# ChunLI-666/PointCloudProcessor

Measured on AMD Instinct MI355X. Metric: Mpoints×frames/sec colorized, higher is better.
Workload: dtype f32/f64

## Files before the change

### include/pcp_hip.h

```cpp
#ifndef PCP_HIP_H
#define PCP_HIP_H

#include <stdint.h>

#ifdef __cplusplus
extern "C" {
#endif

#define PCP_ABI_VERSION 6

#define PCP_OK 0
#define PCP_ERR_INVALID (-1)
#define PCP_ERR_STATE (-2)
#define PCP_ERR_DEVICE (-3)
#define PCP_ERR_NOMEM (-4)
#define PCP_ERR_RANGE (-5)

typedef struct pcp_context pcp_context;

typedef struct pcp_pose {
  double x, y, z, qw, qx, qy, qz;
} pcp_pose;

typedef struct pcp_camera {
// ... 107 lines not shown
int pcp_colour_smooth_local_packed(pcp_context *ctx, float radius, const uint32_t *in_rgba, uint32_t *out_rgba,
                                   int64_t *out_has_count);

int pcp_mls_process(pcp_context *ctx, const pcp_mls_params *p, int64_t *out_count);
int pcp_mls_process_shard(pcp_context *ctx, const pcp_mls_params *p, int64_t index_begin, int64_t index_end,
                          int64_t *out_count);
int pcp_mls_process_slab(pcp_context *ctx, const pcp_mls_params *p, int32_t slab, int32_t n_slabs, int64_t *out_count);
int pcp_mls_stream_begin(pcp_context *ctx, const pcp_mls_params *p, int64_t chunk_capacity, int64_t *out_total,
                         int32_t *out_chunks);
int pcp_mls_stream_next(pcp_context *ctx, int64_t *out_count);
int pcp_mls_stream_seek(pcp_context *ctx, int32_t chunk);
int pcp_mls_fetch(pcp_context *ctx, int64_t capacity, float *out_xyz, float *out_normal, float *out_curvature,
                  int32_t *out_index);
int pcp_cloud_smooth(pcp_context *ctx, const pcp_mls_params *p, int64_t *out_count);

int pcp_cloud_smooth_stream_begin(pcp_context *ctx, const pcp_mls_params *p, int64_t chunk_capacity, int64_t *out_total_rows,
                                  int64_t *out_kept_rows, int32_t *out_chunks);
int pcp_cloud_smooth_stream_next(pcp_context *ctx, int64_t *out_count);
int pcp_cloud_smooth_stream_end(pcp_context *ctx);
int pcp_cloud_smooth_stream_stats(pcp_context *ctx, double out[13]);
int pcp_sor(pcp_context *ctx, int32_t mean_k, double std_mul, uint8_t *out_keep, int64_t *out_kept);
int64_t pcp_sor_chunk_points(void);
int pcp_sor_partial(pcp_context *ctx, int32_t mean_k, int32_t slab, int32_t n_slabs, int64_t capacity, double *out_chunk_sums,
                    int64_t *out_first_chunk, int64_t *out_chunks);
int pcp_sor_finish(pcp_context *ctx, double std_mul, const double *all_chunk_sums, int64_t n_chunks, int32_t slab, int32_t n_slabs,
                   uint8_t *out_keep, int64_t *out_kept);

int pcp_upload_intensity(pcp_context *ctx, const float *intensity, int64_t n);
int pcp_nid_prepare(pcp_context *ctx, int64_t *out_points);
int pcp_nid_evaluate(pcp_context *ctx, const double T[16], const double *T_init, int32_t bins, double *cost,
                     double grad6[6], int32_t *valid);
int pcp_nid_optimize(pcp_context *ctx, const double T_init[16], int32_t bins, int32_t max_outer_iterations,
                     double T_out[16], double *final_cost, int32_t *evaluations);

int pcp_nid_accumulate(pcp_context *ctx, const double T[16], int32_t bins);
int pcp_nid_histograms_device(pcp_context *ctx, void **device_ptr, int64_t *count);
int pcp_nid_finish(pcp_context *ctx, int32_t bins, double *cost, double grad6[6], int32_t *valid);
typedef int (*pcp_nid_eval_fn)(void *user, const double T[16], int32_t bins, double *cost, double grad6[6], int32_t *valid);
int pcp_nid_optimize_with(pcp_context *ctx, pcp_nid_eval_fn eval, void *user, const double T_init[16], int32_t bins,
                          int32_t max_outer_iterations, double T_out[16], double *final_cost, int32_t *evaluations);

int pcp_close_pairs(pcp_context *ctx, double radius, int64_t *points_with_close_neighbour);

int pcp_timing_enable(pcp_context *ctx, int32_t on);
int pcp_timing_reset(pcp_context *ctx);
int pcp_timing_get(pcp_context *ctx, int32_t kernel_id, double *total_ms, int64_t *launches);
const char *pcp_kernel_name(int32_t kernel_id);
int pcp_tile_mask_density(pcp_context *ctx, double *kept_fraction);
int pcp_tile_masks(pcp_context *ctx, int64_t *tiles, int32_t *mask_words, uint32_t *out_words);
int pcp_sor_redo_fraction(pcp_context *ctx, double *fraction);
int pcp_sor_distances(pcp_context *ctx, int64_t capacity, float *out_distance);
int pcp_selftest_arithmetic(pcp_context *ctx, int64_t samples, uint64_t seed, int64_t *mismatches_fp64,
                            int64_t *mismatches_fp32);

#ifdef __cplusplus
}
#endif
#endif
```

### pointcloudprocessor_amd/capi.py

```python
from __future__ import annotations

import ctypes as C
import os
import re

import numpy as np

from . import _build

PCP_OK = 0
PCP_ERR_INVALID = -1
PCP_ERR_STATE = -2
PCP_ERR_DEVICE = -3
PCP_ERR_NOMEM = -4
PCP_ERR_RANGE = -5

NID_EVAL_FN = C.CFUNCTYPE(C.c_int, C.c_void_p, C.POINTER(C.c_double), C.c_int32, C.POINTER(C.c_double), C.POINTER(C.c_double),
                          C.POINTER(C.c_int32))
K_PROJECT, K_DEPTH, K_COLOUR, K_VISIBILITY, K_MLS_GRID, K_MLS_FIT, K_MISC, K_SOR, K_MLS_VOXEL, K_TILE_MASK, K_NID, K_HPR = range(12)
K_COLOUR_SMOOTH = 12
K_COUNT = 13


class PcpError(RuntimeError):
# ... 536 lines not shown
        valid = C.c_int32()
        self._check(self.lib.pcp_nid_finish(self.h, C.c_int32(bins), C.byref(cost), _ptr(grad), C.byref(valid)))
        return cost.value, grad, bool(valid.value)

    def nid_optimize_with(self, evaluate, T_init, bins: int = 16, max_outer_iterations: int = 10):
        errors = []

        @NID_EVAL_FN
        def trampoline(_user, T, b, cost, grad, valid):
            try:
                c, g, ok = evaluate(np.ctypeslib.as_array(T, (16,)).copy().reshape(4, 4), int(b))
                cost[0] = float(c)
                for k in range(6):
                    grad[k] = float(g[k])
                valid[0] = 1 if ok else 0
                return 0
            except Exception as e:
                errors.append(e)
                return -3

        Ti = np.ascontiguousarray(T_init, np.float64).reshape(16)
        out = np.zeros(16, np.float64)
        cost = C.c_double()
        evals = C.c_int32()
        rc = self.lib.pcp_nid_optimize_with(self.h, trampoline, None, _ptr(Ti), C.c_int32(bins), C.c_int32(max_outer_iterations),
                                            _ptr(out), C.byref(cost), C.byref(evals))
        if errors:
            raise errors[0]
        self._check(rc)
        return out.reshape(4, 4), cost.value, evals.value

    def timing_enable(self, on: bool = True):
        self._check(self.lib.pcp_timing_enable(self.h, C.c_int32(1 if on else 0)))

    def timing_reset(self):
        self._check(self.lib.pcp_timing_reset(self.h))

    def timing_get(self, kernel_id: int):
        ms = C.c_double()
        cnt = C.c_int64()
        self._check(self.lib.pcp_timing_get(self.h, C.c_int32(kernel_id), C.byref(ms), C.byref(cnt)))
        return ms.value, cnt.value

    def tile_mask_density(self) -> float:
        v = C.c_double()
        self._check(self.lib.pcp_tile_mask_density(self.h, C.byref(v)))
        return v.value

    def selftest_arithmetic(self, samples: int = 1 << 26, seed: int = 1):
        a, b = C.c_int64(), C.c_int64()
        self._check(self.lib.pcp_selftest_arithmetic(self.h, C.c_int64(samples), C.c_uint64(seed), C.byref(a), C.byref(b)))
        return a.value, b.value

    def tile_masks(self) -> np.ndarray:
        t, w = C.c_int64(), C.c_int32()
        self._check(self.lib.pcp_tile_masks(self.h, C.byref(t), C.byref(w), None))
        out = np.empty((t.value, w.value), np.uint32)
        self._check(self.lib.pcp_tile_masks(self.h, None, None, _ptr(out)))
        return out

    def kernel_name(self, kernel_id: int) -> str:
        return self.lib.pcp_kernel_name(C.c_int32(kernel_id)).decode()
```

### pointcloudprocessor_amd/csrc/pcp_colour.hip

```cpp
#include <algorithm>
#include <cfloat>
#include <cstdlib>

#include "pcp_device.hpp"
#include "pcp_hsv.hpp"
#include "pcp_scan.hpp"

namespace pcp {

constexpr int kBlock = 256;
constexpr uint32_t kFltMaxBits = 0x7f7fffffu;

template <bool kCommon>
__device__ __forceinline__ DevCamera common_camera(const DevCamera &in) {
  DevCamera c = in;
  if constexpr (kCommon) {
    c.cull_mode = PCP_CULL_ZBUFFER;
    c.enable_zbuf = 1;
    c.pretest = 1;
    c.ds_fast = 1;
  }
  return c;
}
inline bool is_common_camera(const DevCamera &c) {
// ... 290 lines not shown
  constexpr uint32_t kXcd = 8, kSuper = kXcd * kXcdChunk;
  const uint32_t b = blockIdx.x;
  if (b >= (gridDim.x / kSuper) * kSuper) return b;
  const uint32_t x = b % kXcd, slot = b / kXcd;
  return ((slot / kXcdChunk) * kXcd + x) * kXcdChunk + slot % kXcdChunk;
}

constexpr unsigned long long kDepthEmpty = 0x7f7f7f7f7f7f7f7full;
__device__ __forceinline__ void depth_min(unsigned long long *__restrict__ map, int32_t cell, unsigned long long bits) {
  if (bits < map[cell]) atomicMin(map + cell, bits);
}
__device__ __forceinline__ double sumsq64(float xc, float yc, float zc) {
  const double X = xc, Y = yc, Z = zc;
  return (X * X + Y * Y) + Z * Z;
}
__global__ __launch_bounds__(kBlock) void k_depth_finish(const unsigned long long *__restrict__ sq, int64_t count,
                                                         uint32_t *__restrict__ range) {
  int64_t i = static_cast<int64_t>(blockIdx.x) * kBlock + threadIdx.x;
  const int64_t stride = static_cast<int64_t>(gridDim.x) * kBlock;
  for (; i < count; i += stride) {
    const unsigned long long b = sq[i];
    float r = FLT_MAX;
    if (b != kDepthEmpty) r = fminf(static_cast<float>(sqrt(__longlong_as_double(static_cast<long long>(b)))), FLT_MAX);
    range[i] = __float_as_uint(r);
  }
}

__device__ __forceinline__ uint32_t range_bits(int32_t w, int32_t f0, int32_t f1) {
  const int32_t fb = max(f0, w << 5), fe = min(f1, (w << 5) + 32);
  const int32_t nb = fe - fb;
  return nb <= 0 ? 0u : (((nb >= 32) ? 0xffffffffu : ((1u << nb) - 1u)) << (fb & 31));
}

template <bool kCommon>
__global__ __launch_bounds__(kBlock) void k_depth_pass(const float *__restrict__ x, const float *__restrict__ y,
                                                       const float *__restrict__ z, int64_t n, DevCamera cam_in,
                                                       const DevFrame *__restrict__ frames, int32_t f0, int32_t f1,
                                                       unsigned long long *__restrict__ depth, int64_t cells,
                                                       int32_t depth_first_frame, uint32_t *__restrict__ tile_mask,
                                                       const uint32_t *__restrict__ tile_inside, int32_t words,
                                                       const int32_t *__restrict__ tile_order) {
  DevCamera cam = common_camera<kCommon>(cam_in);
  if constexpr (kCommon) cam.pretest = 0;
  __shared__ unsigned long long combine[kBlock];
  const int lane = threadIdx.x & 63;
  unsigned long long *tbl = combine + (threadIdx.x & ~63);
  const int64_t j = tile_order ? static_cast<int64_t>(tile_order[blockIdx.x]) * 64 + threadIdx.x
                               : static_cast<int64_t>(xcd_chunked_block()) * kBlock + threadIdx.x;
  const bool live = j < n;
  if (!__ballot(live)) return;
  const float px = live ? x[j] : 0.0f, py = live ? y[j] : 0.0f, pz = live ? z[j] : 0.0f;
  const int64_t tile = __builtin_amdgcn_readfirstlane(static_cast<int32_t>(j >> 6));
  const bool finite_sure = cam.frames_bounded != 0 && __all(fabsf(px) <= 0x1p40f && fabsf(py) <= 0x1p40f && fabsf(pz) <= 0x1p40f);
  unsigned long long *held_at = nullptr;
  unsigned long long held_bits = 0ull, held_seen = 0ull;
  auto settle_held = [&]() {
    if (held_at && held_bits < held_seen) atomicMin(held_at, held_bits);
    held_at = nullptr;
  };
  for (int32_t w = f0 >> 5; w <= (f1 - 1) >> 5; ++w) {
    const uint32_t in_range = range_bits(w, f0, f1);
    uint32_t todo = in_range;
    if (tile_mask) todo &= tile_mask[tile * words + w];
    todo = __builtin_amdgcn_readfirstlane(todo);
    const uint32_t inside = tile_inside ? __builtin_amdgcn_readfirstlane(tile_inside[tile * words + w]) : 0u;
    uint32_t seen = 0u;
    while (todo) {
      const int32_t b = __builtin_ctz(todo);
      const int32_t f = (w << 5) + b;
      todo &= todo - 1u;
      const DevFrame &fr = frames[f];
      const Projected p = project_point(cam, fr.w2c, px, py, pz, ((inside >> b) & 1u) == 0u, finite_sure);
      const bool in_map = live && p.cell >= 0;
      const bool cand = live && p.pixel >= 0 && (cam.enable_zbuf ? p.cell >= 0 : p.cell != -1);
      if (__ballot(cand)) seen |= 1u << b;
      settle_held();
      if (cam.enable_zbuf && __ballot(in_map)) {
        unsigned long long *map = depth + static_cast<uint64_t>(static_cast<uint32_t>(f - depth_first_frame)) * static_cast<uint32_t>(cells);
        unsigned long long key = ~0ull, sbits = 0ull;
        if (in_map) {
          sbits = static_cast<unsigned long long>(__double_as_longlong(sumsq64(p.xc, p.yc, p.zc)));
          key = (static_cast<unsigned long long>(static_cast<uint32_t>(p.cell)) << 32) | (sbits >> 32);
        }
        tbl[lane] = ~0ull;
        __builtin_amdgcn_wave_barrier();
        if (in_map) atomicMin(&tbl[p.cell & 63], key);
        __builtin_amdgcn_wave_barrier();
        if (in_map) {
          const unsigned long long got = tbl[p.cell & 63];
          if (got == key || static_cast<uint32_t>(got >> 32) != static_cast<uint32_t>(p.cell)) {
            held_at = map + p.cell;
            held_bits = sbits;
            held_seen = *held_at;
          }
        }
        __builtin_amdgcn_wave_barrier();
      }
    }
    if (tile_mask && lane == 0 && live) {
      uint32_t *dst = tile_mask + tile * words + w;
      *dst = (*dst & ~in_range) | seen;
    }
  }
  settle_held();
}

__global__ __launch_bounds__(kBlock) void k_visibility(const float *__restrict__ x, const float *__restrict__ y,
                                                       const float *__restrict__ z, int64_t n, DevCamera cam,
                                                       DevFrame fr, const uint32_t *__restrict__ depth,
                                                       const int32_t *__restrict__ perm,
                                                       uint8_t *__restrict__ keep, int32_t require_pixel) {
  const int64_t i = static_cast<int64_t>(blockIdx.x) * kBlock + threadIdx.x;
  if (i >= n) return;
  const Projected p = project_point(cam, fr.w2c, x[i], y[i], z[i]);
  bool k = keep_rule(cam, p, depth);
  if (require_pixel) k = k && p.pixel >= 0;
  if (k) keep[perm ? perm[i] : i] = 1;
}

__device__ __forceinline__ bool keep_by_depth(float xc, float yc, float zc, double lim) {
  const double s = sumsq64(xc, yc, zc);
  const double L = lim * lim;
  bool keep = s < L * (1.0 - 0x1p-40);
  const bool sure = lim > 0.0 && (keep || s > L * (1.0 + 0x1p-40));
  if (!sure) keep = !(sqrt(s) > lim);
  return keep;
}

struct TopState {
  float *score;
  uint32_t *rgb;
  int32_t *frame;
  int32_t *count;
};

struct MatchArgs {
  const uint8_t *in_a;
  unsigned long long *moved;
  float e2;
};

template <bool kCommon, int kMatch, bool kOneShot>
__global__ __launch_bounds__(kBlock) void k_colour_pass(const float *__restrict__ x, const float *__restrict__ y,
                                                        const float *__restrict__ z, int64_t n, DevCamera cam_in,
                                                        const DevFrame *__restrict__ frames, int32_t f0, int32_t f1,
                                                        const uint32_t *__restrict__ depth, int64_t cells,
                                                        const uint32_t *__restrict__ tile_mask, int32_t words,
                                                        const uint32_t *__restrict__ images, int64_t image_px,
                                                        TopState st, const int32_t *__restrict__ perm,
                                                        uint32_t *__restrict__ rgba, int32_t flags_in,
                                                        const uint32_t *__restrict__ hull_bits_in, MatchArgs mb) {
  DevCamera cam = common_camera<kCommon>(cam_in);
  if constexpr (kMatch == 1) cam.match_mode = PCP_MATCH_IDENTITY;
  if constexpr (kMatch == 2 || kMatch == 3) cam.match_mode = PCP_MATCH_ROUNDTRIP;
  const uint32_t *__restrict__ hull_bits = kCommon ? nullptr : hull_bits_in;
  const int32_t flags = kOneShot ? 4 : flags_in;
  const int64_t j = static_cast<int64_t>(xcd_chunked_block()) * kBlock + threadIdx.x;
  const bool live = j < n;
  if (!__ballot(live)) return;
  const float px = live ? x[j] : 0.0f, py = live ? y[j] : 0.0f, pz = live ? z[j] : 0.0f;
  const int64_t tile = __builtin_amdgcn_readfirstlane(static_cast<int32_t>(j >> 6));
  const bool finite_sure = cam.frames_bounded != 0 && __all(fabsf(px) <= 0x1p40f && fabsf(py) <= 0x1p40f && fabsf(pz) <= 0x1p40f);
  Top5 t;
  t.init();
  if ((flags & 1) && live) {
    t.s0 = st.score[0 * n + j]; t.s1 = st.score[1 * n + j]; t.s2 = st.score[2 * n + j];
    t.s3 = st.score[3 * n + j]; t.s4 = st.score[4 * n + j];
    t.c0 = st.rgb[0 * n + j]; t.c1 = st.rgb[1 * n + j]; t.c2 = st.rgb[2 * n + j];
    t.c3 = st.rgb[3 * n + j]; t.c4 = st.rgb[4 * n + j];
    t.f0 = st.frame[0 * n + j]; t.f1 = st.frame[1 * n + j]; t.f2 = st.frame[2 * n + j];
    t.f3 = st.frame[3 * n + j]; t.f4 = st.frame[4 * n + j];
    t.count = st.count[j];
  }
  [[maybe_unused]] bool in_a = false;
  [[maybe_unused]] uint32_t moved = 0u;
  if constexpr (kMatch == 3) in_a = live && mb.in_a[j] != 0;
  for (int32_t w = f0 >> 5; w <= (f1 - 1) >> 5; ++w) {
    uint32_t todo = range_bits(w, f0, f1);
    if (tile_mask) todo &= tile_mask[tile * words + w];
    todo = __builtin_amdgcn_readfirstlane(todo);
    const uint32_t hull_word = (hull_bits && live) ? hull_bits[static_cast<int64_t>(w) * n + j] : 0xffffffffu;
    while (todo) {
      const int32_t f = (w << 5) + __builtin_ctz(todo);
      todo &= todo - 1u;
      const DevFrame &fr = frames[f];
      const Projected p = project_point<false>(cam, fr.w2c, px, py, pz, true, finite_sure);
      const bool cand = live && p.pixel >= 0 && (cam.enable_zbuf ? p.cell >= 0 : p.cell != -1) &&
                        ((hull_word >> (f & 31)) & 1u);
      if (cand) {
        const uint32_t dbits = cam.enable_zbuf ? depth[static_cast<uint64_t>(static_cast<uint32_t>(f)) * static_cast<uint32_t>(cells) + static_cast<uint32_t>(p.cell)] : 0u;
        bool keep = true;
        if (cam.enable_zbuf) keep = keep_by_depth(p.xc, p.yc, p.zc, static_cast<double>(__uint_as_float(dbits)) + cam.slack);
        float sx = p.xc, sy = p.yc, sz = p.zc;
        if constexpr (kMatch == 3) {
          if (keep) keep = roundtrip_sample_moved(cam, fr, px, py, pz, sx, sy, sz, mb.e2, moved) && !in_a;
        } else {
          if (cam.match_mode == PCP_MATCH_ROUNDTRIP && keep) keep = roundtrip_sample(cam, fr, px, py, pz, sx, sy, sz);
        }
        if (keep) {
          const uint32_t texel = images[static_cast<uint64_t>(static_cast<uint32_t>(f)) * static_cast<uint32_t>(image_px) + static_cast<uint32_t>(p.pixel)];
          t.insert(final_score(sx, sy, sz, fr.px, fr.py, fr.pz), texel & 0xffffffu, f);
        }
      }
    }
  }
  if constexpr (kMatch == 3) {
    if (moved) atomicAdd(mb.moved, static_cast<unsigned long long>(moved));
  }
  if (!live) return;
  if (flags & 2) {
    st.score[0 * n + j] = t.s0; st.score[1 * n + j] = t.s1; st.score[2 * n + j] = t.s2;
    st.score[3 * n + j] = t.s3; st.score[4 * n + j] = t.s4;
    st.rgb[0 * n + j] = t.c0; st.rgb[1 * n + j] = t.c1; st.rgb[2 * n + j] = t.c2;
    st.rgb[3 * n + j] = t.c3; st.rgb[4 * n + j] = t.c4;
    st.frame[0 * n + j] = t.f0; st.frame[1 * n + j] = t.f1; st.frame[2 * n + j] = t.f2;
    st.frame[3 * n + j] = t.f3; st.frame[4 * n + j] = t.f4;
    st.count[j] = t.count;
  }
  if (flags & 4) rgba[static_cast<int64_t>(perm[j])] = t.finalise();
}

__global__ __launch_bounds__(kBlock) void k_finalise(int64_t n, TopState st, const int32_t *__restrict__ perm,
                                                     uint32_t *__restrict__ rgba) {
  const int64_t j = static_cast<int64_t>(blockIdx.x) * kBlock + threadIdx.x;
  if (j >= n) return;
  Top5 t;
  t.s0 = st.score[0 * n + j]; t.s1 = st.score[1 * n + j]; t.s2 = st.score[2 * n + j];
  t.s3 = st.score[3 * n + j]; t.s4 = st.score[4 * n + j];
  t.c0 = st.rgb[0 * n + j]; t.c1 = st.rgb[1 * n + j]; t.c2 = st.rgb[2 * n + j];
  t.c3 = st.rgb[3 * n + j]; t.c4 = st.rgb[4 * n + j];
  t.f0 = st.frame[0 * n + j]; t.f1 = st.frame[1 * n + j]; t.f2 = st.frame[2 * n + j];
  t.f3 = st.frame[3 * n + j]; t.f4 = st.frame[4 * n + j];
  t.count = st.count[j];
  rgba[static_cast<int64_t>(perm[j])] = t.finalise();
}

__global__ __launch_bounds__(kBlock) void k_match_fixup(const float *__restrict__ x, const float *__restrict__ y,
                                                        const float *__restrict__ z, int64_t n, DevCamera cam,
                                                        const DevFrame *__restrict__ frames, int32_t f0, int32_t f1,
                                                        const uint32_t *__restrict__ depth, int64_t cells,
                                                        const uint32_t *__restrict__ tile_mask, int32_t words,
                                                        const uint32_t *__restrict__ images, int64_t image_px, TopState st,
                                                        const int32_t *__restrict__ perm, uint32_t *__restrict__ rgba,
                                                        int32_t flags, const uint32_t *__restrict__ hull_bits,
                                                        const int32_t *__restrict__ list, int64_t na,
                                                        const int64_t *__restrict__ off, const int32_t *__restrict__ cols) {
  const int64_t a = static_cast<int64_t>(blockIdx.x) * kBlock + threadIdx.x;
  if (a >= na) return;
  const int64_t j = list[a];
  Top5 t;
  t.init();
  if (flags & 1) {
    t.s0 = st.score[0 * n + j]; t.s1 = st.score[1 * n + j]; t.s2 = st.score[2 * n + j];
// ... 39 lines not shown
  }
  if (flags & 4) rgba[static_cast<int64_t>(perm[j])] = t.finalise();
}

__device__ __forceinline__ uint64_t mix64(uint64_t v) {
  v += 0x9e3779b97f4a7c15ull;
  v = (v ^ (v >> 30)) * 0xbf58476d1ce4e5b9ull;
  v = (v ^ (v >> 27)) * 0x94d049bb133111ebull;
  return v ^ (v >> 31);
}
__device__ __forceinline__ bool same_f64(double a, double b) {
  if (a != a && b != b) return true;
  if (a == 0.0 && b == 0.0) return true;
  return __double_as_longlong(a) == __double_as_longlong(b);
}

__global__ __launch_bounds__(kBlock) void k_selftest_div64(int64_t samples, uint64_t seed,
                                                           unsigned long long *__restrict__ bad) {
  const int64_t i = static_cast<int64_t>(blockIdx.x) * kBlock + threadIdx.x;
  if (i >= samples) return;
  const uint64_t a = mix64(seed ^ static_cast<uint64_t>(i) * 3u), b = mix64(a);
  uint32_t bx = static_cast<uint32_t>(a), by = static_cast<uint32_t>(a >> 32), bz = static_cast<uint32_t>(b);
  const uint32_t mode = static_cast<uint32_t>(b >> 32) & 3u;
  if (mode != 0u) {
    const uint32_t span = mode == 1u ? 12u : 40u;
    bx = (bx & 0x807fffffu) | ((127u - span / 2u + (bx >> 23) % span) << 23);
    by = (by & 0x807fffffu) | ((127u - span / 2u + (by >> 23) % span) << 23);
    bz = (bz & 0x807fffffu) | ((127u - span / 2u + (bz >> 23) % span) << 23);
  }
  const float xc = __uint_as_float(bx), yc = __uint_as_float(by), zc = fabsf(__uint_as_float(bz));
  if (!(zc > 0.0f)) return;
  double xn, yn;
  divide_xy_by_z(xc, yc, zc, xn, yn);
  const double xr = static_cast<double>(xc) / static_cast<double>(zc);
  const double yr = static_cast<double>(yc) / static_cast<double>(zc);
  if (!same_f64(xn, xr) || !same_f64(yn, yr)) atomicAdd(bad, 1ull);
}

__global__ __launch_bounds__(kBlock) void k_selftest_div32(DevCamera cam, unsigned long long *__restrict__ bad) {
  const uint32_t lane = blockIdx.x * kBlock + threadIdx.x;
  uint32_t wrong = 0u;
  for (uint32_t k = 0; k < 256u; ++k) {
    const float x = __uint_as_float((k << 24) | lane);
    const float a = div_by_ds(cam, x), b = x / cam.ds_f;
    const float ax = fabsf(x);
    if (ax >= 0x1p-40f && ax <= 0x1p60f) {
      if (!((a != a && b != b) || __float_as_uint(a) == __float_as_uint(b))) ++wrong;
    } else {
      if (cell_of_quotient(a, cam.cull_wf) != cell_of_quotient(b, cam.cull_wf)) ++wrong;
      if (cell_of_quotient(a, cam.cull_hf) != cell_of_quotient(b, cam.cull_hf)) ++wrong;
    }
  }
  if (wrong) atomicAdd(bad, static_cast<unsigned long long>(wrong));
}

__global__ __launch_bounds__(kBlock) void k_unpack_result(const uint32_t *__restrict__ packed, int64_t n,
                                                         uint8_t *__restrict__ rgb, uint8_t *__restrict__ has) {
  const int64_t i = static_cast<int64_t>(blockIdx.x) * kBlock + threadIdx.x;
  if (i >= n) return;
  const uint32_t v = packed[i];
  rgb[3 * i + 0] = static_cast<uint8_t>(v & 0xffu);
  rgb[3 * i + 1] = static_cast<uint8_t>((v >> 8) & 0xffu);
  rgb[3 * i + 2] = static_cast<uint8_t>((v >> 16) & 0xffu);
  has[i] = static_cast<uint8_t>(v >> 24);
}

__global__ __launch_bounds__(kBlock) void k_fill_u32(uint32_t *__restrict__ p, int64_t n, uint32_t v) {
  int64_t i = static_cast<int64_t>(blockIdx.x) * kBlock + threadIdx.x;
  const int64_t stride = static_cast<int64_t>(gridDim.x) * kBlock;
  for (; i < n; i += stride) p[i] = v;
}

__global__ __launch_bounds__(kBlock) void k_scatter_u32(const uint32_t *__restrict__ in,
                                                        const int32_t *__restrict__ perm, int64_t n,
                                                        uint32_t *__restrict__ out) {
  const int64_t j = static_cast<int64_t>(blockIdx.x) * kBlock + threadIdx.x;
  if (j < n) out[perm[j]] = in[j];
}

__global__ __launch_bounds__(kBlock) void k_pack_bgr(const uint8_t *__restrict__ bgr, int64_t row_stride, int32_t w,
                                                     int32_t h, uint32_t *__restrict__ texels, int32_t clear_mask,
                                                     const int32_t *__restrict__ hsv_tables, float sat_scale,
                                                     float val_scale) {
  const int64_t i = static_cast<int64_t>(blockIdx.x) * kBlock + threadIdx.x;
  if (i >= static_cast<int64_t>(w) * h) return;
  const int32_t v = static_cast<int32_t>(i / w), u = static_cast<int32_t>(i - static_cast<int64_t>(v) * w);
  const uint8_t *p = bgr + static_cast<int64_t>(v) * row_stride + 3 * u;
  const uint32_t keep = clear_mask ? 0u : (texels[i] & 0xff000000u);
  uint32_t b = p[0], g = p[1], r = p[2];
  if (hsv_tables) hsv_round_trip(hsv_tables, hsv_tables + 256, sat_scale, val_scale, b, g, r);
  texels[i] = keep | b | (g << 8) | (r << 16);
}

__global__ __launch_bounds__(kBlock) void k_pack_bgr16(const uint8_t *__restrict__ bgr, int64_t row_stride, int32_t w,
                                                       int32_t h, uint32_t *__restrict__ texels, int32_t clear_mask,
                                                       const int32_t *__restrict__ hsv_tables, float sat_scale,
                                                       float val_scale) {
  const int32_t groups = w >> 4;
  const int64_t n_groups = static_cast<int64_t>(groups) * h;
  const int64_t g = static_cast<int64_t>(blockIdx.x) * kBlock + threadIdx.x;
  uint4 a, b, c;
  if (row_stride == 3 * static_cast<int64_t>(w)) {
    __shared__ uint4 piece[3 * kBlock];
    const int64_t base = static_cast<int64_t>(blockIdx.x) * (3 * kBlock);
    const int64_t pieces = 3 * n_groups;
    const uint4 *src = reinterpret_cast<const uint4 *>(bgr);
// ... 1154 lines not shown
  std::vector<uint32_t> h(static_cast<size_t>(ctx->n_tiles) * ctx->mask_words);
  PCP_HIP_TRY(ctx, hipMemcpyAsync(h.data(), ctx->tile_mask.p, h.size() * 4, hipMemcpyDeviceToHost, ctx->stream));
  PCP_HIP_TRY(ctx, hipStreamSynchronize(ctx->stream));
  uint64_t bits = 0;
  for (uint32_t w : h) bits += static_cast<uint64_t>(__builtin_popcount(w));
  *kept_fraction = static_cast<double>(bits) / (static_cast<double>(ctx->n_tiles) * ctx->n_frames);
  return PCP_OK;
}

int pcp_tile_masks(pcp_context *ctx, int64_t *tiles, int32_t *mask_words, uint32_t *out_words) {
  if (!ctx) return PCP_ERR_INVALID;
  if (!ctx->tile_mask.p || ctx->n_tiles == 0 || ctx->n_frames == 0)
    return set_error(ctx, PCP_ERR_STATE, "pcp_tile_masks: no masks (call pcp_depth_pass)");
  if (tiles) *tiles = ctx->n_tiles;
  if (mask_words) *mask_words = ctx->mask_words;
  if (out_words) {
    PCP_HIP_TRY(ctx, hipMemcpyAsync(out_words, ctx->tile_mask.p, static_cast<size_t>(ctx->n_tiles) * ctx->mask_words * 4,
                                    hipMemcpyDeviceToHost, ctx->stream));
    PCP_HIP_TRY(ctx, hipStreamSynchronize(ctx->stream));
  }
  return PCP_OK;
}

int pcp_colour_result_device(pcp_context *ctx, void **device_ptr, int64_t *n_words) {
  if (!ctx) return PCP_ERR_INVALID;
  if (!ctx->colour_result_live)
    return set_error(ctx, PCP_ERR_STATE, "pcp_colour_result_device: no result (call pcp_colorize / pcp_colour_finalise)");
  if (device_ptr) *device_ptr = ctx->rgba2[ctx->rgba_cur].p;
  if (n_words) *n_words = ctx->n;
  return PCP_OK;
}

int pcp_selftest_arithmetic(pcp_context *ctx, int64_t samples, uint64_t seed, int64_t *mismatches_fp64,
                            int64_t *mismatches_fp32) {
  if (!ctx) return PCP_ERR_INVALID;
  if (!ctx->have_camera) return set_error(ctx, PCP_ERR_STATE, "pcp_selftest_arithmetic: pcp_set_camera has not been called");
  PCP_HIP_TRY(ctx, hipSetDevice(ctx->device));
  if (samples < 0) return set_error(ctx, PCP_ERR_INVALID, "pcp_selftest_arithmetic: negative sample count");
  PCP_HIP_TRY(ctx, ctx->s_counter.ensure(4));
  unsigned long long *bad = ctx->s_counter.p;
  PCP_HIP_TRY(ctx, hipMemsetAsync(bad, 0, 16, ctx->stream));
  if (samples > 0)
    hipLaunchKernelGGL(k_selftest_div64, dim3(blocks_for(samples)), dim3(kBlock), 0, ctx->stream, samples, seed, bad);
  hipLaunchKernelGGL(k_selftest_div32, dim3((1u << 24) / kBlock), dim3(kBlock), 0, ctx->stream, ctx->dcam, bad + 1);
  PCP_HIP_TRY(ctx, hipGetLastError());
  unsigned long long h[2] = {0, 0};
  PCP_HIP_TRY(ctx, hipMemcpyAsync(h, bad, 16, hipMemcpyDeviceToHost, ctx->stream));
  PCP_HIP_TRY(ctx, hipStreamSynchronize(ctx->stream));
  if (mismatches_fp64) *mismatches_fp64 = static_cast<int64_t>(h[0]);
  if (mismatches_fp32) *mismatches_fp32 = static_cast<int64_t>(h[1]);
  return PCP_OK;
}

}
```

### pointcloudprocessor_amd/csrc/pcp_context.hip

```cpp
#include <algorithm>
#include <cfloat>
#include <cmath>
#include <cstdlib>
#include <new>
#include <vector>

#include "pcp_internal.hpp"
#include "pcp_scan.hpp"

namespace pcp {

static thread_local std::string g_error;

int set_error(const pcp_context *ctx, int code, const char *fmt, ...) {
  char buf[1024];
  va_list ap;
  va_start(ap, fmt);
  vsnprintf(buf, sizeof(buf), fmt, ap);
  va_end(ap);
  if (ctx)
    ctx->error = buf;
  else
    g_error = buf;
  return code;
// ... 731 lines not shown
  d.cx = cam->cx;
  d.cy = cam->cy;
  d.k1 = cam->k1;
  d.k2 = cam->k2;
  d.p1 = cam->p1;
  d.p2 = cam->p2;
  d.k3 = cam->k3;
  d.slack = cp.depth_slack;
  d.ds = cp.downsample_factor;
  d.ds_f = static_cast<float>(cp.downsample_factor);
  d.ds_rcp = 1.0f / d.ds_f;
  d.ds_fast = (d.ds_f >= 0x1p-20f && d.ds_f <= 0x1p20f) ? 1 : 0;
  if (const char *e = std::getenv("PCP_DISABLE_FAST_EXACT")) d.ds_fast = (e[0] == '1') ? 0 : d.ds_fast;
  d.img_w = cam->image_width;
  d.img_h = cam->image_height;
  d.cull_w = cam->cull_width;
  d.cull_h = cam->cull_height;
  d.img_wd = static_cast<double>(cam->image_width);
  d.img_hd = static_cast<double>(cam->image_height);
  d.cull_wf = static_cast<float>(cam->cull_width);
  d.cull_hf = static_cast<float>(cam->cull_height);
  d.mw = cam->cull_width / cp.downsample_factor;
  d.mh = cam->cull_height / cp.downsample_factor;
  d.cull_mode = cp.cull_mode == PCP_CULL_HPR ? PCP_CULL_HPR_CANDIDATES : cp.cull_mode;
  d.match_mode = cp.match_mode;
  d.cull_wd = static_cast<double>(cam->cull_width);
  d.cull_hd = static_cast<double>(cam->cull_height);
  {
    const double eps = static_cast<double>(1e-5f);
    d.match_r2 = static_cast<float>(eps * eps);
  }
  d.enable_zbuf = (cp.enable_depth_buffer_culling && cp.cull_mode == PCP_CULL_ZBUFFER) ? 1 : 0;
  d.pretest = 1;
  d.qfx = static_cast<float>(cam->fx);
  d.qfy = static_cast<float>(cam->fy);
  d.qcx = static_cast<float>(cam->cx);
  d.qcy = static_cast<float>(cam->cy);
  d.qk1 = static_cast<float>(cam->k1);
  d.qk2 = static_cast<float>(cam->k2);
  d.qk3 = static_cast<float>(cam->k3);
  d.qp1 = static_cast<float>(cam->p1);
  d.qp2 = static_cast<float>(cam->p2);
  {
    const float ds = static_cast<float>(cp.downsample_factor);
    const bool hpr = cp.cull_mode != PCP_CULL_ZBUFFER;
    const float cw = hpr ? static_cast<float>(d.cull_w) : ds * static_cast<float>(d.enable_zbuf ? d.mw : d.cull_w);
    const float ch = hpr ? static_cast<float>(d.cull_h) : ds * static_cast<float>(d.enable_zbuf ? d.mh : d.cull_h);
    d.u_lo = -(ds + 0.5f);
    d.v_lo = -(ds + 0.5f);
    d.u_hi = std::max(cw, static_cast<float>(d.img_w)) + 0.5f;
    d.v_hi = std::max(ch, static_cast<float>(d.img_h)) + 0.5f;
  }
  if (const char *e = std::getenv("PCP_DISABLE_PRETEST")) d.pretest = (e[0] == '1') ? 0 : 1;

  ctx->have_camera = true;
  for (hipStream_t us : ctx->upload_stream)
    if (us) (void)hipStreamSynchronize(us);
  std::fill(ctx->image_pending.begin(), ctx->image_pending.end(), uint8_t(0));
  ctx->image_set.assign(ctx->image_set.size(), 0);
  ctx->mask_set.assign(ctx->mask_set.size(), 0);
  std::fill(ctx->depth_valid.begin(), ctx->depth_valid.end(), uint8_t(0));
  ctx->hull_valid.clear();
  ctx->colour_state_live = false;
  ctx->colour_result_live = false;
  return PCP_OK;
}

int pcp_upload_cloud(pcp_context *ctx, const float *x, const float *y, const float *z, int64_t n) {
  if (!ctx) return PCP_ERR_INVALID;
  if (n < 0 || n >= (int64_t(1) << 31)) return set_error(ctx, PCP_ERR_INVALID, "pcp_upload_cloud: n=%lld out of range", (long long)n);
  if (n > 0 && (!x || !y || !z)) return set_error(ctx, PCP_ERR_INVALID, "pcp_upload_cloud: NULL coordinate array");
  return store_cloud(ctx, x, y, z, n);
}

int pcp_upload_cloud_aos(pcp_context *ctx, const void *points, int64_t n, int64_t stride_bytes) {
  if (!ctx) return PCP_ERR_INVALID;
  if (n < 0 || n >= (int64_t(1) << 31)) return set_error(ctx, PCP_ERR_INVALID, "pcp_upload_cloud_aos: n out of range");
  if (stride_bytes < 12) return set_error(ctx, PCP_ERR_INVALID, "pcp_upload_cloud_aos: stride must be >= 12 bytes");
  if (n > 0 && !points) return set_error(ctx, PCP_ERR_INVALID, "pcp_upload_cloud_aos: NULL points");
  if (stride_bytes % 4 == 0 && (reinterpret_cast<uintptr_t>(points) & 3u) == 0)
    return store_cloud(ctx, nullptr, nullptr, nullptr, n, points, stride_bytes);
  std::vector<float> x(static_cast<size_t>(n)), y(static_cast<size_t>(n)), z(static_cast<size_t>(n));
  const uint8_t *base = static_cast<const uint8_t *>(points);
  for (int64_t i = 0; i < n; ++i) {
    float v[3];
    std::memcpy(v, base + i * stride_bytes, 12);
    x[static_cast<size_t>(i)] = v[0];
    y[static_cast<size_t>(i)] = v[1];
    z[static_cast<size_t>(i)] = v[2];
  }
  return store_cloud(ctx, x.data(), y.data(), z.data(), n);
}

int64_t pcp_cloud_size(const pcp_context *ctx) { return ctx ? ctx->n : -1; }

int pcp_pose_to_matrices(const pcp_pose *pose, const double *T_opt, float w2c[12], float c2w[12]) {
  if (!pose || !w2c || !c2w) {
    set_global_error("pcp_pose_to_matrices: NULL argument");
    return PCP_ERR_INVALID;
  }
  matrices_from_pose(*pose, T_opt, w2c, c2w);
  return PCP_OK;
}

int pcp_set_frames(pcp_context *ctx, const pcp_pose *poses, int32_t n_frames, const double *T_opt,
                   int32_t T_opt_stride) {
// ... 90 lines not shown
```

### pointcloudprocessor_amd/csrc/pcp_device.hpp

```cpp
#pragma once

#include <hip/hip_runtime.h>

#include <cfloat>
#include <cstdint>

#include "pcp_internal.hpp"

namespace pcp {

__device__ __forceinline__ void xform(const float *__restrict__ m, float x, float y, float z, float &xc, float &yc,
                                      float &zc) {
  xc = x * m[0] + (y * m[1] + (z * m[2] + m[3]));
  yc = x * m[4] + (y * m[5] + (z * m[6] + m[7]));
  zc = x * m[8] + (y * m[9] + (z * m[10] + m[11]));
}

__device__ __forceinline__ void divide_xy_by_z(float xc, float yc, float zc, double &xn, double &yn, bool finite_sure = false) {
  const double X = xc, Y = yc, Z = zc;
  if (finite_sure || (xc - xc) + (yc - yc) + (zc - zc) == 0.0f) {
    double r = __builtin_amdgcn_rcp(Z);
    double e = __builtin_fma(-Z, r, 1.0);
    r = __builtin_fma(r, e, r);
    e = __builtin_fma(-Z, r, 1.0);
// ... 50 lines not shown
  return ((q > -1.0f) & (q < size)) ? static_cast<int32_t>(q) : -1;
}

template <bool kShortDiv = true>
__device__ __forceinline__ int32_t cull_cell(const DevCamera &c, double u, double v) {
  if (c.cull_mode == PCP_CULL_HPR_CANDIDATES) {
    return (u > -1.0 && u < c.cull_wd && v > -1.0 && v < c.cull_hd) ? -2 : -1;
  }
  const float cxf = kShortDiv ? div_by_ds(c, static_cast<float>(u)) : static_cast<float>(u) / c.ds_f;
  const float cyf = kShortDiv ? div_by_ds(c, static_cast<float>(v)) : static_cast<float>(v) / c.ds_f;
  const int32_t cx = cell_of_quotient(cxf, c.cull_wf), cy = cell_of_quotient(cyf, c.cull_hf);
  if ((cx < 0) | (cy < 0)) return -1;
  return ((cx < c.mw) & (cy < c.mh)) ? cy * c.mw + cx : (c.enable_zbuf ? -1 : -2);
}

__device__ __forceinline__ int32_t colour_pixel(const DevCamera &c, double u, double v) {
  if (!(u > -1.0 && u < c.img_wd && v > -1.0 && v < c.img_hd)) return -1;
  return static_cast<int32_t>(v) * c.img_w + static_cast<int32_t>(u);
}

__device__ __forceinline__ double range64(float xc, float yc, float zc) {
  const double X = xc, Y = yc, Z = zc;
  return sqrt((X * X + Y * Y) + Z * Z);
}

__device__ __forceinline__ bool surely_rejected(const DevCamera &c, float xc, float yc, float zc) {
  const float rz = __builtin_amdgcn_rcpf(zc);
  const float xn = xc * rz, yn = yc * rz;
  const float x2 = xn * xn, y2 = yn * yn;
  const float r2 = x2 + y2, r4 = r2 * r2, r6 = r2 * r4;
  const float rc = __builtin_fmaf(c.qk3, r6, __builtin_fmaf(c.qk2, r4, __builtin_fmaf(c.qk1, r2, 1.0f)));
  const float ra = __builtin_fmaf(fabsf(c.qk3), r6, __builtin_fmaf(fabsf(c.qk2), r4, __builtin_fmaf(fabsf(c.qk1), r2, 1.0f)));
  const float t1 = 2.0f * xn * yn;
  const float t2 = __builtin_fmaf(2.0f, x2, r2), t3 = __builtin_fmaf(2.0f, y2, r2);
  const float at1 = fabsf(t1);
  const float xd = __builtin_fmaf(c.qp2, t2, __builtin_fmaf(c.qp1, t1, rc * xn));
  const float yd = __builtin_fmaf(c.qp2, t1, __builtin_fmaf(c.qp1, t3, rc * yn));
  const float sx = __builtin_fmaf(fabsf(c.qp2), t2, __builtin_fmaf(fabsf(c.qp1), at1, ra * fabsf(xn)));
  const float sy = __builtin_fmaf(fabsf(c.qp2), at1, __builtin_fmaf(fabsf(c.qp1), t3, ra * fabsf(yn)));
  const float u = __builtin_fmaf(c.qfx, xd, c.qcx), v = __builtin_fmaf(c.qfy, yd, c.qcy);
  constexpr float kErr = 1.52587890625e-05f;
  const float eu = kErr * __builtin_fmaf(fabsf(c.qfx), sx, fabsf(c.qcx));
  const float ev = kErr * __builtin_fmaf(fabsf(c.qfy), sy, fabsf(c.qcy));
  const float over = fmaxf(fmaxf(c.u_lo - (u + eu), (u - eu) - c.u_hi), fmaxf(c.v_lo - (v + ev), (v - ev) - c.v_hi));
  return over > 0.0f;
}

struct Projected {
  float xc, yc, zc;
  int32_t cell;
  int32_t pixel;
};

template <bool kPretest = true, bool kShortDiv = true>
__device__ __forceinline__ Projected project_point(const DevCamera &c, const float *__restrict__ m, float x, float y,
                                                   float z, bool pretest_here = true, bool finite_sure = false) {
  Projected p;
  xform(m, x, y, z, p.xc, p.yc, p.zc);
  p.cell = -1;
  p.pixel = -1;
  if (p.zc > 0.0f && !(kPretest && pretest_here && c.pretest && surely_rejected(c, p.xc, p.yc, p.zc))) {
    double u, v;
    project_uv<kShortDiv>(c, p.xc, p.yc, p.zc, u, v, finite_sure);
    p.cell = cull_cell<kShortDiv>(c, u, v);
    p.pixel = colour_pixel(c, u, v);
  }
  return p;
}

__device__ __forceinline__ bool keep_rule(const DevCamera &c, const Projected &p, const uint32_t *__restrict__ depth) {
  if (!c.enable_zbuf) return p.cell != -1;
  if (p.cell < 0) return false;
  const double r = range64(p.xc, p.yc, p.zc);
  const double lim = static_cast<double>(__uint_as_float(depth[p.cell])) + c.slack;
  return !(r > lim);
}

__device__ __forceinline__ bool roundtrip_sample(const DevCamera &c, const DevFrame &fr, float wx0, float wy0, float wz0,
                                                 float &xc, float &yc, float &zc) {
  float wx, wy, wz;
  xform(fr.c2w, xc, yc, zc, wx, wy, wz);
  const float dx = wx - wx0, dy = wy - wy0, dz = wz - wz0;
  float d2 = dx * dx;
  d2 += dy * dy;
  d2 += dz * dz;
  if (!(d2 < c.match_r2)) return false;
  const float *m = fr.c2w_inv;
  xc = (m[0] * wx + m[1] * wy) + (m[2] * wz + m[3]);
  yc = (m[4] * wx + m[5] * wy) + (m[6] * wz + m[7]);
  zc = (m[8] * wx + m[9] * wy) + (m[10] * wz + m[11]);
  return true;
}

__device__ __forceinline__ bool roundtrip_sample_moved(const DevCamera &c, const DevFrame &fr, float wx0, float wy0, float wz0,
                                                       float &xc, float &yc, float &zc, float e2, uint32_t &moved) {
  float wx, wy, wz;
  xform(fr.c2w, xc, yc, zc, wx, wy, wz);
  const float dx = wx - wx0, dy = wy - wy0, dz = wz - wz0;
  float d2 = dx * dx;
  d2 += dy * dy;
  d2 += dz * dz;
  moved += (d2 <= e2) ? 0u : 1u;
  if (!(d2 < c.match_r2)) return false;
  const float *m = fr.c2w_inv;
  xc = (m[0] * wx + m[1] * wy) + (m[2] * wz + m[3]);
  yc = (m[4] * wx + m[5] * wy) + (m[6] * wz + m[7]);
  zc = (m[8] * wx + m[9] * wy) + (m[10] * wz + m[11]);
  return true;
}

__device__ __forceinline__ float final_score(float xc, float yc, float zc, double px, double py, double pz) {
  const double dx = static_cast<double>(xc) - px;
  const double dy = static_cast<double>(yc) - py;
  const double dz = static_cast<double>(zc) - pz;
  const double sq = (dx * dx + dy * dy) + dz * dz;
  const double y0 = __builtin_amdgcn_rsq(sq);
  const double e = __builtin_fma(-(sq * y0), y0, 1.0);
  const double y = __builtin_fma(y0 * e, __builtin_fma(0.375, e, 0.5), y0);
  const double t = (dz * y + 1.0) * 0.5;
  const float lo = static_cast<float>(t - 4e-15), hi = static_cast<float>(t + 4e-15);
// ... 79 lines not shown
```

### pointcloudprocessor_amd/csrc/pcp_internal.hpp

```cpp
#pragma once

#include <hip/hip_runtime.h>

#include <cstdarg>
#include <cstdint>
#include <chrono>
#include <cstdio>
#include <cstring>
#include <string>
#include <vector>

#include "pcp_hip.h"

namespace pcp {

struct DevCamera {
  double fx, fy, cx, cy;
  double k1, k2, p1, p2, k3;
  double slack;
  float ds_f;
  double img_wd, img_hd;
  float cull_wf, cull_hf;
  float ds_rcp;
  int32_t ds_fast;
  int32_t ds;
  int32_t img_w, img_h;
  int32_t cull_w, cull_h;
  int32_t mw, mh;
  int32_t enable_zbuf;
  int32_t cull_mode;
  int32_t match_mode;
  double cull_wd, cull_hd;
  float match_r2;
  int32_t pretest;
  int32_t frames_bounded;
  float qfx, qfy, qcx, qcy;
  float qk1, qk2, qk3, qp1, qp2;
  float u_lo, u_hi, v_lo, v_hi;
};

struct DevFrame {
  float w2c[12];
  float c2w[12];
  double px, py, pz;
  double norm_bound;
  float c2w_inv[12];
  float pad_[4];
};
static_assert(sizeof(DevFrame) == 192, "DevFrame layout");

constexpr int kTopM = 5;

struct TimingSlot {
  double total_ms = 0.0;
  int64_t launches = 0;
};

struct PendingEvent {
  hipEvent_t start, stop;
  int32_t kernel;
};

struct AllocTally {
  double seconds = 0.0, bytes = 0.0;
};
inline AllocTally &alloc_tally() {
  static AllocTally t;
  return t;
}
struct AllocClock {
  std::chrono::steady_clock::time_point t0 = std::chrono::steady_clock::now();
  ~AllocClock() { alloc_tally().seconds += std::chrono::duration<double>(std::chrono::steady_clock::now() - t0).count(); }
};

template <typename T>
struct DevBuf {
  T *p = nullptr;
  size_t count = 0;
  hipError_t ensure(size_t n) {
    if (n <= count && p) return hipSuccess;
    AllocClock clk;
    if (p) (void)hipFree(p);
    p = nullptr;
    count = 0;
    if (n == 0) return hipSuccess;
    hipError_t e = hipMalloc(reinterpret_cast<void **>(&p), n * sizeof(T));
    if (e == hipSuccess) {
      count = n;
      alloc_tally().bytes += static_cast<double>(n) * sizeof(T);
    }
    return e;
// ... 275 lines not shown
```

Before: 1.833 million.

## Add certified fp32 projection fast path with fp64 fallback in colour kernels

Adds an fp32 projection with a rigorous error bound that decides the cull cell and colour pixel in single precision. It falls back to the fp64 projection only when the bound straddles a cell or pixel boundary, and the pixel index is recomputed in fp64 only when needed. The aim is to remove most fp64 divides and distortion math from the per-point, per-frame inner loop of the depth and colour passes. It adds a projection self-test entry point and extra camera constants, and relies on the correctness of the hand-derived error bounds.

```diff
diff --git a/include/pcp_hip.h b/include/pcp_hip.h
--- a/include/pcp_hip.h
+++ b/include/pcp_hip.h
@@ -183,6 +183,8 @@
 int pcp_sor_distances(pcp_context *ctx, int64_t capacity, float *out_distance);
 int pcp_selftest_arithmetic(pcp_context *ctx, int64_t samples, uint64_t seed, int64_t *mismatches_fp64,
                             int64_t *mismatches_fp32);
+int pcp_selftest_projection(pcp_context *ctx, int64_t samples, uint64_t seed, int64_t *wrong, int64_t *unsure,
+                            int64_t *pixel_open);
 
 #ifdef __cplusplus
 }
diff --git a/pointcloudprocessor_amd/capi.py b/pointcloudprocessor_amd/capi.py
--- a/pointcloudprocessor_amd/capi.py
+++ b/pointcloudprocessor_amd/capi.py
@@ -612,6 +612,12 @@
         self._check(self.lib.pcp_selftest_arithmetic(self.h, C.c_int64(samples), C.c_uint64(seed), C.byref(a), C.byref(b)))
         return a.value, b.value
 
+    def selftest_projection(self, samples: int = 1 << 24, seed: int = 1):
+        w, u, p = C.c_int64(), C.c_int64(), C.c_int64()
+        self._check(self.lib.pcp_selftest_projection(self.h, C.c_int64(samples), C.c_uint64(seed), C.byref(w), C.byref(u),
+                                                     C.byref(p)))
+        return w.value, u.value, p.value
+
     def tile_masks(self) -> np.ndarray:
         t, w = C.c_int64(), C.c_int32()
         self._check(self.lib.pcp_tile_masks(self.h, C.byref(t), C.byref(w), None))
diff --git a/pointcloudprocessor_amd/csrc/pcp_colour.hip b/pointcloudprocessor_amd/csrc/pcp_colour.hip
--- a/pointcloudprocessor_amd/csrc/pcp_colour.hip
+++ b/pointcloudprocessor_amd/csrc/pcp_colour.hip
@@ -366,6 +366,7 @@
   const float px = live ? x[j] : 0.0f, py = live ? y[j] : 0.0f, pz = live ? z[j] : 0.0f;
   const int64_t tile = __builtin_amdgcn_readfirstlane(static_cast<int32_t>(j >> 6));
   const bool finite_sure = cam.frames_bounded != 0 && __all(fabsf(px) <= 0x1p40f && fabsf(py) <= 0x1p40f && fabsf(pz) <= 0x1p40f);
+  const bool certified = kCommon && finite_sure && cam.fast_proj != 0;
   unsigned long long *held_at = nullptr;
   unsigned long long held_bits = 0ull, held_seen = 0ull;
   auto settle_held = [&]() {
@@ -384,7 +385,9 @@
       const int32_t f = (w << 5) + b;
       todo &= todo - 1u;
       const DevFrame &fr = frames[f];
-      const Projected p = project_point(cam, fr.w2c, px, py, pz, ((inside >> b) & 1u) == 0u, finite_sure);
+      bool pixel_exact;
+      const Projected p = certified ? project_point_certified<false>(cam, fr.w2c, px, py, pz, pixel_exact)
+                                    : project_point(cam, fr.w2c, px, py, pz, ((inside >> b) & 1u) == 0u, finite_sure);
       const bool in_map = live && p.cell >= 0;
       const bool cand = live && p.pixel >= 0 && (cam.enable_zbuf ? p.cell >= 0 : p.cell != -1);
       if (__ballot(cand)) seen |= 1u << b;
@@ -475,6 +478,7 @@
   const float px = live ? x[j] : 0.0f, py = live ? y[j] : 0.0f, pz = live ? z[j] : 0.0f;
   const int64_t tile = __builtin_amdgcn_readfirstlane(static_cast<int32_t>(j >> 6));
   const bool finite_sure = cam.frames_bounded != 0 && __all(fabsf(px) <= 0x1p40f && fabsf(py) <= 0x1p40f && fabsf(pz) <= 0x1p40f);
+  const bool certified = kCommon && finite_sure && cam.fast_proj != 0;
   Top5 t;
   t.init();
   if ((flags & 1) && live) {
@@ -498,7 +502,9 @@
       const int32_t f = (w << 5) + __builtin_ctz(todo);
       todo &= todo - 1u;
       const DevFrame &fr = frames[f];
-      const Projected p = project_point<false>(cam, fr.w2c, px, py, pz, true, finite_sure);
+      bool pixel_exact = true;
+      const Projected p = certified ? project_point_certified<true>(cam, fr.w2c, px, py, pz, pixel_exact)
+                                    : project_point<false>(cam, fr.w2c, px, py, pz, true, finite_sure);
       const bool cand = live && p.pixel >= 0 && (cam.enable_zbuf ? p.cell >= 0 : p.cell != -1) &&
                         ((hull_word >> (f & 31)) & 1u);
       if (cand) {
@@ -512,7 +518,8 @@
           if (cam.match_mode == PCP_MATCH_ROUNDTRIP && keep) keep = roundtrip_sample(cam, fr, px, py, pz, sx, sy, sz);
         }
         if (keep) {
-          const uint32_t texel = images[static_cast<uint64_t>(static_cast<uint32_t>(f)) * static_cast<uint32_t>(image_px) + static_cast<uint32_t>(p.pixel)];
+          const int32_t pixel = pixel_exact ? p.pixel : max(exact_pixel(cam, p), 0);
+          const uint32_t texel = images[static_cast<uint64_t>(static_cast<uint32_t>(f)) * static_cast<uint32_t>(image_px) + static_cast<uint32_t>(pixel)];
           t.insert(final_score(sx, sy, sz, fr.px, fr.py, fr.pz), texel & 0xffffffu, f);
         }
       }
@@ -658,6 +665,66 @@
     }
   }
   if (wrong) atomicAdd(bad, static_cast<unsigned long long>(wrong));
+}
+
+__device__ __forceinline__ double edge_target(const DevCamera &c, uint64_t h, int32_t w, int32_t m) {
+  const uint32_t kind = static_cast<uint32_t>(h) % 4u;
+  double t;
+  if (kind == 0u) t = static_cast<double>(static_cast<int32_t>((h >> 8) % static_cast<uint64_t>(w + 40)) - 20);
+  else if (kind == 1u) t = static_cast<double>(static_cast<int32_t>((h >> 8) % static_cast<uint64_t>(m + 4)) - 2) * c.ds;
+  else if (kind == 2u) t = ((h >> 8) & 1u) ? -1.0 : static_cast<double>(w);
+  else t = ((h >> 8) & 1u) ? -static_cast<double>(c.ds) : static_cast<double>(m) * c.ds;
+  const double offs[4] = {0.0, 1e-6, 1e-4, 1e-2};
+  const double o = offs[(h >> 40) & 3u];
+  return t + (((h >> 42) & 1u) ? o : -o);
+}
+__device__ __forceinline__ double invert_axis(double fx, double cx, double t) { return (t - cx) / fx; }
+__global__ __launch_bounds__(kBlock) void k_selftest_projection(DevCamera cam_in, int64_t samples, uint64_t seed,
+                                                                unsigned long long *__restrict__ bad) {
+  const DevCamera cam = common_camera<true>(cam_in);
+  const int64_t i = static_cast<int64_t>(blockIdx.x) * kBlock + threadIdx.x;
+  if (i >= samples) return;
+  const uint64_t a = mix64(seed ^ (static_cast<uint64_t>(i) * 0x9e3779b97f4a7c15ull)), b = mix64(a), d = mix64(b);
+  const uint32_t mode = static_cast<uint32_t>(d >> 60);
+  const double ua = static_cast<double>(a >> 11) * 0x1p-53, va = static_cast<double>(b >> 11) * 0x1p-53;
+  double xn = (ua - 0.5) * 4.0, yn = (va - 0.5) * 4.0;
+  if (mode >= 6u) {
+    const bool aim_u = mode != 15u, aim_v = mode >= 11u;
+    double tu = aim_u ? edge_target(cam, a, cam.img_w, cam.mw) : cam.fx * (ua - 0.5) * 2.0 + cam.cx;
+    double tv = aim_v ? edge_target(cam, b, cam.img_h, cam.mh) : cam.fy * (va - 0.5) * 2.0 + cam.cy;
+    xn = invert_axis(cam.fx, cam.cx, tu);
+    yn = invert_axis(cam.fy, cam.cy, tv);
+    for (int it = 0; it < 2; ++it) {
+      double u, v;
+      const double x2 = xn * xn, y2 = yn * yn, r2 = x2 + y2;
+      const double rc = ((1.0 + cam.k1 * r2) + cam.k2 * r2 * r2) + cam.k3 * r2 * r2 * r2;
+      const double xd = (rc * xn + cam.p1 * (2.0 * xn * yn)) + cam.p2 * (r2 + 2.0 * x2);
+      const double yd = (rc * yn + cam.p1 * (r2 + 2.0 * y2)) + cam.p2 * (2.0 * xn * yn);
+      u = cam.fx * xd + cam.cx;
+      v = cam.fy * yd + cam.cy;
+      const double drc = 2.0 * cam.k1 + 4.0 * cam.k2 * r2 + 6.0 * cam.k3 * r2 * r2;
+      const double jx = cam.fx * (rc + drc * x2 + 2.0 * cam.p1 * yn + 6.0 * cam.p2 * xn);
+      const double jy = cam.fy * (rc + drc * y2 + 6.0 * cam.p1 * yn + 2.0 * cam.p2 * xn);
+      if (jx != 0.0) xn -= (u - tu) / jx;
+      if (jy != 0.0) yn -= (v - tv) / jy;
+    }
+  }
+  const double lz = static_cast<double>((d >> 8) & 0xffffffull) * 0x1p-24;
+  const double zc64 = mode < 3u ? pow(10.0, -6.0 + 4.0 * lz) : pow(10.0, -2.0 + 6.0 * lz);
+  const float zc = static_cast<float>(zc64), xc = static_cast<float>(xn * zc64), yc = static_cast<float>(yn * zc64);
+  if (!(zc > 0.0f)) return;
+  int32_t cell, pixel;
+  bool pixel_exact;
+  const bool sure = certified_project<true>(cam, xc, yc, zc, cell, pixel, pixel_exact);
+  if (!sure) {
+    atomicAdd(bad + 1, 1ull);
+    return;
+  }
+  double u, v;
+  project_uv<true>(cam, xc, yc, zc, u, v, true);
+  const int32_t cell64 = cull_cell<true>(cam, u, v), pixel64 = colour_pixel(cam, u, v);
+  if (cell != cell64 || (pixel >= 0) != (pixel64 >= 0) || (pixel_exact && pixel != pixel64)) atomicAdd(bad, 1ull);
+  if (!pixel_exact && pixel64 >= 0) atomicAdd(bad + 2, 1ull);
 }
 
 __global__ __launch_bounds__(kBlock) void k_unpack_result(const uint32_t *__restrict__ packed, int64_t n,
@@ -1918,4 +1985,27 @@
   return PCP_OK;
 }
 
-}
+int pcp_selftest_projection(pcp_context *ctx, int64_t samples, uint64_t seed, int64_t *wrong, int64_t *unsure,
+                            int64_t *pixel_open) {
+  if (!ctx) return PCP_ERR_INVALID;
+  if (!ctx->have_camera) return set_error(ctx, PCP_ERR_STATE, "pcp_selftest_projection: pcp_set_camera has not been called");
+  PCP_HIP_TRY(ctx, hipSetDevice(ctx->device));
+  if (samples < 0) return set_error(ctx, PCP_ERR_INVALID, "pcp_selftest_projection: negative sample count");
+  if (!ctx->dcam.fast_proj || !ctx->dcam.ds_fast || ctx->cull.cull_mode != PCP_CULL_ZBUFFER || !ctx->dcam.enable_zbuf)
+    return set_error(ctx, PCP_ERR_INVALID, "pcp_selftest_projection: the camera is outside the certified configuration");
+  PCP_HIP_TRY(ctx, ctx->s_counter.ensure(4));
+  unsigned long long *bad = ctx->s_counter.p;
+  PCP_HIP_TRY(ctx, hipMemsetAsync(bad, 0, 24, ctx->stream));
+  if (samples > 0)
+    hipLaunchKernelGGL(k_selftest_projection, dim3(blocks_for(samples)), dim3(kBlock), 0, ctx->stream, ctx->dcam, samples, seed, bad);
+  PCP_HIP_TRY(ctx, hipGetLastError());
+  unsigned long long h[3] = {0, 0, 0};
+  PCP_HIP_TRY(ctx, hipMemcpyAsync(h, bad, 24, hipMemcpyDeviceToHost, ctx->stream));
+  PCP_HIP_TRY(ctx, hipStreamSynchronize(ctx->stream));
+  if (wrong) *wrong = static_cast<int64_t>(h[0]);
+  if (unsure) *unsure = static_cast<int64_t>(h[1]);
+  if (pixel_open) *pixel_open = static_cast<int64_t>(h[2]);
+  return PCP_OK;
+}
+
+}
diff --git a/pointcloudprocessor_amd/csrc/pcp_context.hip b/pointcloudprocessor_amd/csrc/pcp_context.hip
--- a/pointcloudprocessor_amd/csrc/pcp_context.hip
+++ b/pointcloudprocessor_amd/csrc/pcp_context.hip
@@ -807,6 +807,25 @@
     d.v_hi = std::max(ch, static_cast<float>(d.img_h)) + 0.5f;
   }
   if (const char *e = std::getenv("PCP_DISABLE_PRETEST")) d.pretest = (e[0] == '1') ? 0 : 1;
+  {
+    auto small = [](double v) { return std::isfinite(v) && std::fabs(v) <= 0x1p30; };
+    const bool ok = small(cam->fx) && small(cam->fy) && small(cam->cx) && small(cam->cy) && small(cam->k1) &&
+                    small(cam->k2) && small(cam->k3) && small(cam->p1) && small(cam->p2) && cp.downsample_factor >= 1 &&
+                    cp.downsample_factor <= (1 << 20) && cam->image_width <= (1 << 24) && cam->image_height <= (1 << 24);
+    d.fast_proj = ok ? 1 : 0;
+    auto up = [](double v) { return std::nextafter(static_cast<float>(v), INFINITY); };
+    constexpr double u = 0x1p-24;
+    const double F = std::max(std::fabs(static_cast<double>(d.qfx)), std::fabs(static_cast<double>(d.qfy)));
+    const double Cc = std::max(std::fabs(static_cast<double>(d.qcx)), std::fabs(static_cast<double>(d.qcy)));
+    d.fe_a = up(14.0 * u * F);
+    d.fe_b = up(42.0 * u * F);
+    d.fe_p = up(static_cast<double>(d.fe_b) * 3.0 * (std::fabs(static_cast<double>(d.qp1)) + std::fabs(static_cast<double>(d.qp2))));
+    d.fe_c = up(8.0 * u * Cc + 0x1p-60);
+    d.img_wf = static_cast<float>(d.img_w);
+    d.img_hf = static_cast<float>(d.img_h);
+    d.mw_f = d.mw > 0 ? static_cast<float>(d.mw) : -1.0f;
+    d.mh_f = d.mh > 0 ? static_cast<float>(d.mh) : -1.0f;
+  }
 
   ctx->have_camera = true;
   for (hipStream_t us : ctx->upload_stream)
diff --git a/pointcloudprocessor_amd/csrc/pcp_device.hpp b/pointcloudprocessor_amd/csrc/pcp_device.hpp
--- a/pointcloudprocessor_amd/csrc/pcp_device.hpp
+++ b/pointcloudprocessor_amd/csrc/pcp_device.hpp
@@ -126,6 +126,50 @@
   int32_t pixel;
 };
 
+typedef float f32x2 __attribute__((ext_vector_type(2)));
+__device__ __forceinline__ f32x2 fma2(f32x2 a, f32x2 b, f32x2 c) { return __builtin_elementwise_fma(a, b, c); }
+template <bool kPixelIndex>
+__device__ __forceinline__ bool certified_project(const DevCamera &c, float xc, float yc, float zc, int32_t &cell,
+                                                  int32_t &pixel, bool &pixel_exact) {
+  const float rz = __builtin_amdgcn_rcpf(zc);
+  const f32x2 n = f32x2{xc, yc} * rz;
+  const f32x2 sq = n * n;
+  const float r2 = sq.x + sq.y, r4 = r2 * r2, r6 = r2 * r4;
+  const float dk = __builtin_fmaf(c.qk3, r6, __builtin_fmaf(c.qk2, r4, c.qk1 * r2));
+  const float ak = __builtin_fmaf(fabsf(c.qk3), r6, __builtin_fmaf(fabsf(c.qk2), r4, fabsf(c.qk1) * r2));
+  const float t1 = 2.0f * n.x * n.y;
+  const f32x2 t23 = fma2(sq, f32x2{2.0f, 2.0f}, f32x2{r2, r2});
+  f32x2 d = fma2(f32x2{dk, dk}, n, n);
+  d = fma2(f32x2{c.qp1, c.qp1}, f32x2{t1, t23.y}, d);
+  d = fma2(f32x2{c.qp2, c.qp2}, f32x2{t23.x, t1}, d);
+  const f32x2 uv = fma2(f32x2{c.qfx, c.qfy}, d, f32x2{c.qcx, c.qcy});
+  const float g = __builtin_fmaf(c.fe_b, ak, c.fe_a), h = __builtin_fmaf(c.fe_p, r2, c.fe_c);
+  const f32x2 e = fma2(f32x2{fabsf(n.x), fabsf(n.y)}, f32x2{g, g}, f32x2{h, h});
+  const f32x2 lo = uv - e, hi = uv + e;
+  const f32x2 ql = lo * c.ds_rcp, qh = hi * c.ds_rcp;
+  const f32x2 mq = ql - f32x2{floorf(qh.x), floorf(qh.y)};
+  const f32x2 a = uv + 1.0f, b = f32x2{c.img_wf, c.img_hf} - uv;
+  const f32x2 mp = f32x2{fminf(fabsf(a.x), fabsf(b.x)), fminf(fabsf(a.y), fabsf(b.y))} - e;
+  const float margin = fminf(fminf(mq.x, mq.y), fminf(mp.x, mp.y));
+  const bool sure = (margin > 0.0f) & ((fabsf(uv.x) + fabsf(uv.y)) + (e.x + e.y) <= FLT_MAX);
+  if constexpr (kPixelIndex) {
+    const f32x2 mi = lo - f32x2{floorf(hi.x), floorf(hi.y)};
+    pixel_exact = fminf(mi.x, mi.y) > 0.0f;
+  } else {
+    pixel_exact = false;
+  }
+  const f32x2 q = uv * c.ds_rcp;
+  const f32x2 qa = q + 1.0f, qb = f32x2{c.mw_f, c.mh_f} - q;
+  const float in_map = fminf(fminf(qa.x, qb.x), fminf(qa.y, qb.y));
+  cell = in_map > 0.0f ? static_cast<int32_t>(q.y) * c.mw + static_cast<int32_t>(q.x) : -1;
+  const bool in_image = fminf(fminf(a.x, b.x), fminf(a.y, b.y)) > 0.0f;
+  if constexpr (kPixelIndex)
+    pixel = in_image ? static_cast<int32_t>(uv.y) * c.img_w + static_cast<int32_t>(uv.x) : -1;
+  else
+    pixel = in_image ? 0 : -1;
+  return sure;
+}
+
 template <bool kPretest = true, bool kShortDiv = true>
 __device__ __forceinline__ Projected project_point(const DevCamera &c, const float *__restrict__ m, float x, float y,
                                                    float z, bool pretest_here = true, bool finite_sure = false) {
@@ -140,6 +184,29 @@
     p.pixel = colour_pixel(c, u, v);
   }
   return p;
+}
+
+template <bool kPixelIndex>
+__device__ __forceinline__ Projected project_point_certified(const DevCamera &c, const float *__restrict__ m, float x,
+                                                             float y, float z, bool &pixel_exact) {
+  Projected p;
+  xform(m, x, y, z, p.xc, p.yc, p.zc);
+  p.cell = -1;
+  p.pixel = -1;
+  pixel_exact = true;
+  if (p.zc > 0.0f && !certified_project<kPixelIndex>(c, p.xc, p.yc, p.zc, p.cell, p.pixel, pixel_exact)) {
+    double u, v;
+    project_uv<true>(c, p.xc, p.yc, p.zc, u, v, true);
+    p.cell = cull_cell<true>(c, u, v);
+    p.pixel = colour_pixel(c, u, v);
+    pixel_exact = true;
+  }
+  return p;
+}
+__device__ __forceinline__ int32_t exact_pixel(const DevCamera &c, const Projected &p) {
+  double u, v;
+  project_uv<true>(c, p.xc, p.yc, p.zc, u, v, true);
+  return colour_pixel(c, u, v);
 }
 
 __device__ __forceinline__ bool keep_rule(const DevCamera &c, const Projected &p, const uint32_t *__restrict__ depth) {
diff --git a/pointcloudprocessor_amd/csrc/pcp_internal.hpp b/pointcloudprocessor_amd/csrc/pcp_internal.hpp
--- a/pointcloudprocessor_amd/csrc/pcp_internal.hpp
+++ b/pointcloudprocessor_amd/csrc/pcp_internal.hpp
@@ -37,6 +37,10 @@
   float qfx, qfy, qcx, qcy;
   float qk1, qk2, qk3, qp1, qp2;
   float u_lo, u_hi, v_lo, v_hi;
+  int32_t fast_proj;
+  float fe_a, fe_b, fe_p, fe_c;
+  float img_wf, img_hf;
+  float mw_f, mh_f;
 };
 
 struct DevFrame {
```

After: 1.768 million (median of 6 runs). -3.5%, worse.
